# cv-stuttgart/PCFA

Measured on AMD Instinct MI355X. Metric: attack_steps_per_sec, higher is better.
Workload: dtype f32; 1 GPU; RAFT, 1 synthetic 436x1024 pair per GPU (padded 440x1024), disjoint delta, change_of_variables, delta_bound=0.005, zero target, L-BFGS max_iter=10; weights=random:1234, parallelism=pairs sharded 1/GPU, closure_launch=hipGraph replay

## Files before the change

include/pcfa_hip.h:

```cpp
#ifndef PCFA_HIP_H
#define PCFA_HIP_H

#include <stddef.h>
#include <stdint.h>

#ifdef __cplusplus
extern "C" {
#endif

#define PCFA_OK 0
#define PCFA_ERR_INVALID_ARG (-1)
#define PCFA_ERR_UNSUPPORTED (-2)
#define PCFA_ERR_WORKSPACE (-3)

#if defined(__GNUC__)
#define PCFA_API __attribute__((visibility("default")))
#else
#define PCFA_API
#endif

#define PCFA_MAX_LEVELS 8
#define PCFA_ABI_VERSION 3

#define PCFA_LOSS_AEE 0
// ... 224 lines not shown

PCFA_API int pcfa_sepconv5_gru_gates_fwd(const float* h, int C, const float* rest, int Cr, const float* w_packed,
                                const float* add_zr, float* z, float* r, float* rh, int B, int H, int W,
                                int vertical, void* stream);
PCFA_API int pcfa_sepconv5_gru_update_fwd(const float* rh, int C, const float* rest, int Cr, const float* w_packed,
                                 const float* add_q, const float* z, const float* h, float* q, float* hnew, int B,
                                 int H, int W, int vertical, void* stream);
PCFA_API int pcfa_sepconv5_gru_gates_bwd(const float* dqc, int C, int Cr, const float* w_packed_bwd, const float* z,
                                const float* r, const float* h, const float* dz, const float* dh_in, float* dzr,
                                float* dh, float* d_rest, int accumulate_rest, int B, int H, int W, int vertical,
                                void* stream);
PCFA_API int pcfa_sepconv5_gru_update_bwd(const float* dzr, int C, int Cr, const float* w_packed_bwd, const float* dh_acc,
                                 const float* z_prev, const float* q_prev, const float* h_prev, float* dz_prev,
                                 float* dqc_prev, float* dh_prev, float* d_rest, int B, int H, int W, int vertical,
                                 void* stream);

PCFA_API long long pcfa_conv3x3_packed_floats(int K, int N);
PCFA_API int pcfa_conv3x3_pack_weights(const float* w, float* fwd_packed, float* bwd_packed, int Cout, int Cin,
                              void* stream);
PCFA_API int pcfa_conv3x3_fwd(const float* x, const float* packed, const float* bias, float* out, int B, int K, int N,
                     int H, int W, int relu, void* stream);
PCFA_API int pcfa_conv3x3_act_fwd(const float* x, const float* packed, const float* bias, float* out, int B, int K,
                         int N, int H, int W, int act, float slope, void* stream);
PCFA_API int pcfa_leaky_relu_fwd(const float* x, float* y, float slope, long long n, void* stream);
PCFA_API int pcfa_leaky_relu_bwd(const float* out, const float* grad_out, float* grad_x, float slope, long long n,
                        void* stream);
PCFA_API int pcfa_conv3x3_act_fwd_pair(const float* x, const float* packed, const float* bias, float* out, int K, int N,
                              const float* x2, const float* packed2, const float* bias2, float* out2, int K2, int N2,
                              int H, int W, int act, float slope, void* stream);
PCFA_API int pcfa_conv3x3_fused_bwd(const float* g, const float* packed_bwd, const float* mask, const float* addend,
// ... 162 lines not shown
```

pcfa_amd/_hip.py:

```python
import ctypes
import os
from ctypes import c_char_p, c_double, c_float, c_int, c_longlong, c_size_t, c_uint, c_ulonglong, c_void_p, POINTER

ABI_VERSION = 3
LIB_PATH = os.environ.get("PCFA_HIP_LIB") or os.path.join(os.path.dirname(os.path.abspath(__file__)), "lib",
                                                          "libpcfa_hip.so")

PCFA_LOSS = {"aee": 0, "mse": 1, "cosim": 2}


class HipLibraryError(RuntimeError):
    pass


_P = c_void_p
_S4 = POINTER(c_longlong)

SIGNATURES = {
    "pcfa_abi_version": (c_int, []),
    "pcfa_timing_arm": (c_int, [_P, _P, c_int]),
    "pcfa_null_launch": (c_int, [_P]),
    "pcfa_poison_lds": (c_int, [c_uint, _P]),
    "pcfa_peek_lds": (c_int, [_P, c_int, _P]),
    "pcfa_calib_mfma_f32": (c_longlong, [_P, c_int, c_int, _P]),
# ... 79 lines not shown
    "pcfa_sepconv5_algo": (c_int, [c_int]),
    "pcfa_sepconv5_uses_winograd": (c_int, [c_int] * 7),
    "pcfa_sepconv5_pack_weights": (c_int, [_P, _P, _P, c_int, c_int, _P]),
    "pcfa_sepconv5_fwd": (c_int, [_P, c_int, _P, c_int, _P, _P, c_int, c_int, c_int, c_int, c_int, _P]),
    "pcfa_sepconv5_fwd_split": (c_int, [_P, c_int, _P, c_int, _P, _P, c_int, c_int, _P, c_int, c_int, c_int, c_int, c_int,
                                        c_int, _P]),
    "pcfa_gru_gates_bwd_acc": (c_int, [_P, _P, _P, _P, _P, _P, _P, _P, _P, c_longlong, _P]),
    "pcfa_sepconv5_fwd_split_masked": (c_int, [_P, c_int, _P, c_int, _P, _P, c_int, c_int, _P, c_int, _P, c_int, c_int,
                                               c_int, c_int, c_int, c_int, _P]),
    "pcfa_sepconv5_gru_gates_fwd": (c_int, [_P, c_int, _P, c_int, _P, _P, _P, _P, _P, c_int, c_int, c_int, c_int, _P]),
    "pcfa_sepconv5_gru_update_fwd": (c_int, [_P, c_int, _P, c_int, _P, _P, _P, _P, _P, _P, c_int, c_int, c_int, c_int, _P]),
    "pcfa_sepconv5_gru_gates_bwd": (c_int, [_P, c_int, c_int, _P, _P, _P, _P, _P, _P, _P, _P, _P, c_int, c_int, c_int,
                                            c_int, c_int, _P]),
    "pcfa_sepconv5_gru_update_bwd": (c_int, [_P, c_int, c_int, _P, _P, _P, _P, _P, _P, _P, _P, _P, c_int, c_int, c_int,
                                             c_int, _P]),
    "pcfa_convex_upsample_fwd": (c_int, [_P, _P, _P, c_int, c_int, c_int, _P]),
    "pcfa_convex_upsample_workspace_floats": (c_longlong, [c_int, c_int, c_int]),
    "pcfa_convex_upsample_bwd": (c_int, [_P, _P, _P, _P, _P, _P, c_int, c_int, c_int, _P]),
    "pcfa_flow_step": (c_int, [_P, _P, _P, _P, _P, c_longlong, _P]),
    "pcfa_conv3x3_act_fwd_pair": (c_int, [_P, _P, _P, _P, c_int, c_int, _P, _P, _P, _P, c_int, c_int, c_int, c_int, c_int,
                                          c_float, _P]),
    "pcfa_relu_bwd2": (c_int, [_P, _P, _P, _P, _P, c_longlong, _P]),
    "pcfa_conv3x3_fused_bwd": (c_int, [_P, _P, _P, _P, _P, c_int, c_int, c_int, c_int, c_int, _P]),
    "pcfa_conv3x3_masked_fwd": (c_int, [_P, _P, _P, _P, c_int, c_int, c_int, c_int, c_int, _P]),
    "pcfa_conv3x3_algo": (c_int, [c_int] * 5),
    "pcfa_conv3x3_workspace_bytes": (c_size_t, [c_int] * 5),
    "pcfa_conv3x3_run": (c_int, [_P] * 6 + [c_int] * 6 + [c_float, c_int, _P, c_size_t, _P]),
    "pcfa_conv3x3_run_strided": (c_int, [_P, c_longlong, _P, _P, _P, c_longlong, _P, c_longlong, _P, c_longlong]
                                 + [c_int] * 6 + [c_float, c_int, _P, c_size_t, _P]),
    "pcfa_conv3x3_packed_floats": (c_longlong, [c_int, c_int]),
# ... 126 lines not shown
```

pcfa_amd/csrc/gru_math.hip:

```cpp
#include "common.hpp"

namespace {

__device__ __forceinline__ float sigmoidf_(float x) { return 1.0f / (1.0f + expf(-x)); }

template <typename F>
__device__ __forceinline__ void for_each4(long long n, int vec_ok, F f) {
  const long long stride = (long long)gridDim.x * blockDim.x;
  const long long gid = (long long)blockIdx.x * blockDim.x + threadIdx.x;
  if (!vec_ok) {
    for (long long i = gid; i < n; i += stride) f(i, false);
    return;
  }
  const long long n4 = n >> 2;
  for (long long i = gid; i < n4; i += stride) f(i, true);
  if (blockIdx.x == 0 && threadIdx.x < (n & 3)) f((n4 << 2) + threadIdx.x, false);
}

#define LD4(p, i) (*reinterpret_cast<const float4*>((p) + ((i) << 2)))
#define ST4(p, i, v) (*reinterpret_cast<float4*>((p) + ((i) << 2)) = (v))

__device__ __forceinline__ float bias_at(const float* __restrict__ b, long long e, int plane, int C) {
  return b ? b[(e / plane) % C] : 0.f;
}
// ... 80 lines not shown
      o.w = (1.f - zz.w) * hh.w + zz.w * qq.w;
      ST4(q, i, qq); ST4(hnew, i, o);
    } else {
      const float qq = tanhf(qc[i] + (aq ? aq[i] : 0.f) + bias_at(bq, i, plane, C));
      q[i] = qq;
      hnew[i] = (1.f - z[i]) * h[i] + z[i] * qq;
    }
  });
}

__global__ void gru_update_bwd_kernel(const float* __restrict__ z, const float* __restrict__ q,
                                      const float* __restrict__ h, const float* __restrict__ g,
                                      float* __restrict__ dz, float* __restrict__ dqc,
                                      float* __restrict__ dh, long long n, int vec_ok) {
  auto one = [](float z_, float q_, float h_, float g_, float& a, float& b, float& c) {
    a = g_ * q_ - g_ * h_;
    b = (g_ * z_) * (1.f - q_ * q_);
    c = g_ * (1.f - z_);
  };
  for_each4(n, vec_ok, [&](long long i, bool vec) {
    if (vec) {
      const float4 zz = LD4(z, i), qq = LD4(q, i), hh = LD4(h, i), gg = LD4(g, i);
      float4 a, b, c;
      one(zz.x, qq.x, hh.x, gg.x, a.x, b.x, c.x);
      one(zz.y, qq.y, hh.y, gg.y, a.y, b.y, c.y);
      one(zz.z, qq.z, hh.z, gg.z, a.z, b.z, c.z);
      one(zz.w, qq.w, hh.w, gg.w, a.w, b.w, c.w);
      ST4(dz, i, a); ST4(dqc, i, b); ST4(dh, i, c);
    } else {
      one(z[i], q[i], h[i], g[i], dz[i], dqc[i], dh[i]);
    }
  });
}
// ... 199 lines not shown
```

pcfa_amd/csrc/sepconv5.hpp:

```cpp
#pragma once
#include "common.hpp"

namespace pcfa_sc5 {

struct Operand {
  const float* a;
  const float* b;
  int Ca, Cin;
};

struct OutSplit {
  float* a;
  float* b;
  int Ca;
  int acc_a, acc_b;
  const float* mask_b;
  int mask_cb;
};

struct GruEpi {
  int mode, C;
  const float* p0;
  const float* p1;
  const float* p2;
  const float* p3;
  const float* p4;
  float* o0;
  float* o1;
  float* o2;
};

constexpr int PCFA_SC5_NOT_ELIGIBLE = -12345;
int sc5_wino_enabled(int set);
bool sc5_wino_shape_ok(int B, int Cin, int Ca, int Cout, int H, int W, int vertical);
long long sc5_wino_packed_floats(int Cout, int Cin);
int sc5_wino_pack(const float* w, float* packed, int Cout, int Cin, int transpose, hipStream_t stream);
int sc5_wino_launch(const Operand& in, const float* w_wino, const OutSplit& out, int B, int Cout, int H, int W,
                    int vertical, hipStream_t stream, const GruEpi& epi);

}
```

pcfa_amd/csrc/sepconv5_wino.hip:

```cpp
#include <cstdlib>
#include "sepconv5.hpp"

#ifndef PCFA_SC5W_DBG
#define PCFA_SC5W_DBG 0
#endif
#ifndef PCFA_SC5W_WLDS
#define PCFA_SC5W_WLDS 1
#endif
#ifndef PCFA_SC5W_STORE_AT
#define PCFA_SC5W_STORE_AT 1
#endif

namespace {
using namespace pcfa_sc5;

typedef float f32x16 __attribute__((ext_vector_type(16)));
typedef float f32x4 __attribute__((ext_vector_type(4)));
typedef float f32x2 __attribute__((ext_vector_type(2)));

constexpr int CK = 8, STEPS = (CK / 2) * 6;
constexpr int HPX = 128, HRV = HPX / 4 + 2, HCHS = 4 * HRV, HPATCH = CK * HCHS, HNV = CK * HRV;
constexpr int VPX = 64, VCHS = 6 * 64, VPATCH = CK * VCHS, VNV = CK * 6 * 16;

__device__ __attribute__((aligned(16))) float sc5_zero_piece[4] = {0.f, 0.f, 0.f, 0.f};

__device__ __forceinline__ float wino_sigmoid(float x) { return 1.0f / (1.0f + expf(-x)); }

__device__ __forceinline__ const float* wino_plane(const Operand& in, int ci, long long plane) {
  return ci < in.Ca ? in.a + ci * plane : in.b + (ci - in.Ca) * plane;
}

__global__ void sc5_wino_pack_kernel(const float* __restrict__ w, float* __restrict__ P, int N, int C, int transpose,
                                     long long total) {
  const double G[6][5] = {{0.25, 0., 0., 0., 0.},
                          {-1. / 6, -1. / 6, -1. / 6, -1. / 6, -1. / 6},
                          {-1. / 6, 1. / 6, -1. / 6, 1. / 6, -1. / 6},
                          {1. / 24, 2. / 24, 4. / 24, 8. / 24, 16. / 24},
                          {1. / 24, -2. / 24, 4. / 24, -8. / 24, 16. / 24},
                          {0., 0., 0., 0., 1.}};
// ... 5 lines not shown
    const int n = 32 * nb + (lane & 31), c = chunk * CK + 2 * (s / 6) + (lane >> 5), i = s % 6;
    double u = 0.0;
    if (n < N && c < C)
      for (int t = 0; t < 5; ++t)
        u += G[i][t] * (double)(transpose ? w[((long long)c * N + n) * 5 + (4 - t)] : w[((long long)n * C + c) * 5 + t]);
    P[e] = (float)u;
  }
}

template <bool VERT, int WN, int KS, int MODE>
__global__ __launch_bounds__(128 * WN * KS) void sc5_wino_kernel(Operand in, const float* __restrict__ wp, OutSplit out,
                                                                 int Cout, int H, int W, int tiles_x, GruEpi epi) {
  constexpr int GT = 128 * WN, WPG = 2 * WN;
  constexpr int PATCH = VERT ? VPATCH : HPATCH, NV = VERT ? VNV : HNV, NLOAD = (NV + GT - 1) / GT;
  constexpr int RN = 16 / KS;
  constexpr int WBLK = STEPS * 64;
  extern __shared__ __attribute__((aligned(16))) float smem_all[];
  const int grp = __builtin_amdgcn_readfirstlane(threadIdx.x / GT);
  float* smem = smem_all + grp * 2 * PATCH;
  float* wlds = smem_all + KS * 2 * PATCH + grp * 2 * WN * WBLK;
  const int tid = threadIdx.x % GT, lane = tid & 63, l31 = lane & 31, lh = lane >> 5;
  const int wv = __builtin_amdgcn_readfirstlane(tid >> 6);
  const int wn = WN == 2 ? (wv & 1) : 0, wpx = WN == 2 ? (wv >> 1) : wv;
  const int ty = blockIdx.x / tiles_x, x0 = (blockIdx.x - ty * tiles_x) * (VERT ? VPX : HPX);
  const int nb = blockIdx.y * WN + wn;
  const long long plane = (long long)H * W;
  const int nchunk_all = in.Cin / CK, nchunk = nchunk_all / KS;
  in.a += (long long)blockIdx.z * in.Ca * plane;
  if (in.b) in.b += (long long)blockIdx.z * (in.Cin - in.Ca) * plane;
  out.a += (long long)blockIdx.z * out.Ca * plane;
  if (out.b) out.b += (long long)blockIdx.z * (Cout - out.Ca) * plane;
  if (out.mask_b) out.mask_b += (long long)blockIdx.z * (Cout - out.Ca) * plane;

  int poff[NLOAD], pch[NLOAD], plds[NLOAD];
  unsigned okm = 0;
#pragma unroll
  for (int k = 0; k < NLOAD; ++k) {
    const int e = min(tid + GT * k, NV - 1);
    if (VERT) {
      const int c = e / 96, rem = e - c * 96, r = rem >> 4, v = rem & 15;
      const int iy = 2 * ty - 2 + r;
      okm |= (unsigned)((int)(iy >= 0) & (int)(iy < H)) << k;
      poff[k] = min(max(iy, 0), H - 1) * W + x0 + 4 * v;
      pch[k] = c;
      plds[k] = c * VCHS + r * 64 + 4 * v;
    } else {
      const int c = e / HRV, v = e - c * HRV;
// ... 15 lines not shown
      const f32x4 zero = {0.f, 0.f, 0.f, 0.f};
      const f32x4 t = (okm >> k & 1u) ? rr[k] : zero;
      if (tid + GT * k < NV) *reinterpret_cast<f32x4*>(smem + buf * PATCH + plds[k]) = t;
    }
  };
  auto dma_patch = [&](int chunk, int buf) {
#pragma unroll
    for (int k = 0; k < NLOAD; ++k) {
      const float* src = (okm >> k & 1u) ? wino_plane(in, (KS * chunk + grp) * CK + pch[k], plane) + poff[k] : sc5_zero_piece;
      float* dst = smem + buf * PATCH + 4 * (GT * k + 64 * wv);
      if (tid + GT * k < NV)
        __builtin_amdgcn_global_load_lds((const __attribute__((address_space(1))) void*)src,
                                         (__attribute__((address_space(3))) void*)dst, 16, 0, 0);
    }
  };
  const float* pw = wp + ((long long)nb * nchunk_all * STEPS) * 64;

  f32x16 acc[6];
#pragma unroll
  for (int i = 0; i < 6; ++i)
#pragma unroll
    for (int r = 0; r < 16; ++r) acc[i][r] = 0.f;

  f32x4 ra[NLOAD], rb[NLOAD];
  float wa[STEPS], wb[STEPS];
  if (PCFA_SC5W_WLDS) dma_patch(0, 0);
  else load_patch(0, ra);
  auto load_w = [&](int chunk_global, float (&w)[STEPS]) {
    const f32x4* q4 = reinterpret_cast<const f32x4*>(pw + (long long)chunk_global * STEPS * 64);
#pragma unroll
    for (int sq = 0; sq < STEPS / 4; ++sq) {
      const f32x4 t = q4[sq * 64 + lane];
      w[4 * sq] = t.x;
      w[4 * sq + 1] = t.y;
      w[4 * sq + 2] = t.z;
      w[4 * sq + 3] = t.w;
    }
  };
  auto dma_w = [&](int chunk_global, int slot) {
    const float* src = pw + (long long)chunk_global * WBLK + (3 * wpx * 64 + lane) * 4;
    float* dst = wlds + (slot * WN + wn) * WBLK + 3 * wpx * 256;
#pragma unroll
    for (int k = 0; k < 3; ++k)
      __builtin_amdgcn_global_load_lds((const __attribute__((address_space(1))) void*)(src + k * 256),
                                       (__attribute__((address_space(3))) void*)(dst + k * 256), 16, 0, 0);
  };
  auto read_w = [&](int slot, int sq, float (&w)[STEPS]) {
    const f32x4 t = *reinterpret_cast<const f32x4*>(wlds + (slot * WN + wn) * WBLK + (sq * 64 + lane) * 4);
    w[4 * sq] = t.x;
    w[4 * sq + 1] = t.y;
    w[4 * sq + 2] = t.z;
    w[4 * sq + 3] = t.w;
  };
  if (PCFA_SC5W_WLDS) {
    dma_w(grp, 0);
    dma_w(KS * min(1, nchunk - 1) + grp, 1);
  } else {
    load_w(grp, wa);
  }

  const int mw = 32 * nb;
  const bool rowB = !VERT || 2 * ty + 1 < H;
  const long long pix = VERT ? (long long)(2 * ty) * W + x0 + 32 * wpx + l31 : (long long)ty * W + x0 + 64 * wpx + 2 * l31;
  const long long pixB = VERT ? (rowB ? W : 0) : 1;
  const int RB = grp * RN;
  auto ld2 = [&](const float* p, long long idx) -> f32x2 {
    if (!VERT) return *reinterpret_cast<const f32x2*>(p + idx);
    f32x2 v = {p[idx], p[idx + pixB]};
    return v;
  };
  auto st2 = [&](float* p, long long idx, float a, float b) {
    if (!VERT) {
      f32x2 v = {a, b};
      *reinterpret_cast<f32x2*>(p + idx) = v;
    } else {
      p[idx] = a;
      if (rowB) p[idx + W] = b;
    }
  };
  auto ml_of = [&](int rr) { const int r = RB + rr; return (r & 3) + 8 * (r >> 2) + 4 * lh; };

  const bool apart = mw < epi.C;
  f32x2 e0[RN], e1[RN], e2[RN], e3[RN], e4[RN];
#pragma unroll
  for (int rr = 0; rr < RN; ++rr) e0[rr] = e1[rr] = e2[rr] = e3[rr] = e4[rr] = (f32x2){0.f, 0.f};
  if (MODE == 1) {
    const long long ia0 = ((long long)blockIdx.z * 2 * epi.C + mw) * plane + pix;
    const long long ic0 = ((long long)blockIdx.z * epi.C + (apart ? mw : mw - epi.C)) * plane + pix;
#pragma unroll
    for (int rr = 0; rr < RN; ++rr) {
      e0[rr] = ld2(epi.p0, ia0 + ml_of(rr) * plane);
      e1[rr] = ld2(epi.p1, ic0 + ml_of(rr) * plane);
    }
  } else if (MODE == 2) {
    const long long ic0 = ((long long)blockIdx.z * epi.C + mw) * plane + pix;
#pragma unroll
    for (int rr = 0; rr < RN; ++rr) {
      e0[rr] = ld2(epi.p0, ic0 + ml_of(rr) * plane);
      e1[rr] = ld2(epi.p1, ic0 + ml_of(rr) * plane);
      e2[rr] = ld2(epi.p2, ic0 + ml_of(rr) * plane);
    }
  } else if (MODE >= 3) {
    if (apart) {
      const long long ic0 = ((long long)blockIdx.z * epi.C + mw) * plane + pix;
#pragma unroll
      for (int rr = 0; rr < RN; ++rr) {
        e0[rr] = ld2(epi.p0, ic0 + ml_of(rr) * plane);
        e1[rr] = ld2(epi.p1, ic0 + ml_of(rr) * plane);
        e2[rr] = ld2(epi.p2, ic0 + ml_of(rr) * plane);
        e3[rr] = ld2(epi.p3, ic0 + ml_of(rr) * plane);
        if (MODE == 3 && epi.p4 != nullptr) e4[rr] = ld2(epi.p4, ic0 + ml_of(rr) * plane);
      }
    }
  }

  if (PCFA_SC5W_WLDS) asm volatile("s_waitcnt vmcnt(0)" ::: "memory");
  else store_patch(0, ra);
  __syncthreads();
  if (PCFA_SC5W_WLDS) {
#pragma unroll
    for (int sq = 0; sq < STEPS / 4; ++sq) read_w(0, sq, wa);
    __syncthreads();
  } else {
    load_patch(min(1, nchunk - 1), rb);
  }

  const int bl = VERT ? lh * VCHS + 32 * wpx + l31 : lh * HCHS + 2 * (32 * wpx + l31) + 2;
  constexpr int CHS = VERT ? VCHS : HCHS;

// ... 53 lines not shown
          read_w((chunk + 1) & 1, 2 * p + 1, wnext);
        } else {
          read_w((chunk + 1) & 1, p + 2, wnext);
        }
      }
      if (!PCFA_SC5W_WLDS && p == PCFA_SC5W_STORE_AT && !(PCFA_SC5W_DBG & 16)) store_patch((chunk + 1) & 1, rstore);
      __builtin_amdgcn_sched_barrier(0);
    }
    if (!PCFA_SC5W_WLDS && PCFA_SC5W_STORE_AT >= CK / 2 && !(PCFA_SC5W_DBG & 16)) store_patch((chunk + 1) & 1, rstore);
    if (PCFA_SC5W_WLDS) {
      __builtin_amdgcn_sched_barrier(0);
      asm volatile("s_waitcnt vmcnt(0)" ::: "memory");
    }
    if (!(PCFA_SC5W_DBG & 1)) __syncthreads();
  };
  for (int chunk = 0; chunk < nchunk; chunk += 2) {
    item(chunk, wa, wb, ra, rb);
    item(chunk + 1, wb, wa, rb, ra);
  }

  float* sred = smem_all;
#pragma unroll
  for (int r = 0; r < 16; ++r) {
    const float s12 = acc[1][r] + acc[2][r], d12 = acc[1][r] - acc[2][r], s34 = acc[3][r] + acc[4][r],
                d34 = acc[3][r] - acc[4][r];
    sred[((grp * WPG + wv) * 32 + r) * 64 + lane] = acc[0][r] + s12 + s34;
    sred[((grp * WPG + wv) * 32 + 16 + r) * 64 + lane] = fmaf(2.f, d34, d12) + acc[5][r];
  }
  __syncthreads();
  float ya[RN], yb[RN];
#pragma unroll
  for (int rr = 0; rr < RN; ++rr) {
    float sa = 0.f, sb = 0.f;
#pragma unroll
    for (int g = 0; g < KS; ++g) {
      sa += sred[((g * WPG + wv) * 32 + RB + rr) * 64 + lane];
      sb += sred[((g * WPG + wv) * 32 + 16 + RB + rr) * 64 + lane];
    }
    ya[rr] = sa;
    yb[rr] = sb;
  }

  if (MODE == 1) {
    const long long io0 = ((long long)blockIdx.z * epi.C + (apart ? mw : mw - epi.C)) * plane + pix;
#pragma unroll
    for (int rr = 0; rr < RN; ++rr) {
      const long long io = io0 + ml_of(rr) * plane;
      const float sa = wino_sigmoid(ya[rr] + e0[rr].x), sb = wino_sigmoid(yb[rr] + e0[rr].y);
      if (apart) {
        st2(epi.o0, io, sa, sb);
      } else {
        st2(epi.o1, io, sa, sb);
        st2(epi.o2, io, sa * e1[rr].x, sb * e1[rr].y);
      }
    }
  } else if (MODE == 2) {
// ... 20 lines not shown
        const float dr = drh_ * h_;
        ob[q] = dr * (1.f - r_) * r_;
        float c = drh_ * r_;
        if (epi.p4 != nullptr) c += q ? e4[rr].y : e4[rr].x;
        oc[q] = c;
      }
      st2(epi.o0, j0 + ml * plane, oa[0], oa[1]);
      st2(epi.o1, j0 + (long long)(epi.C + ml) * plane, ob[0], ob[1]);
      st2(epi.o2, i0 + ml * plane, oc[0], oc[1]);
    }
  } else if (MODE == 4 && apart) {
    const long long i0 = ((long long)blockIdx.z * epi.C + mw) * plane + pix;
#pragma unroll
    for (int rr = 0; rr < RN; ++rr) {
      const long long i = i0 + ml_of(rr) * plane;
      float oa[2], ob[2], oc[2];
#pragma unroll
      for (int q = 0; q < 2; ++q) {
        const float g_ = (q ? e0[rr].y : e0[rr].x) + (q ? yb[rr] : ya[rr]);
        const float z_ = q ? e1[rr].y : e1[rr].x, q_ = q ? e2[rr].y : e2[rr].x, h_ = q ? e3[rr].y : e3[rr].x;
        oa[q] = g_ * q_ - g_ * h_;
        ob[q] = (g_ * z_) * (1.f - q_ * q_);
        oc[q] = g_ * (1.f - z_);
      }
      st2(epi.o0, i, oa[0], oa[1]);
      st2(epi.o1, i, ob[0], ob[1]);
      st2(epi.o2, i, oc[0], oc[1]);
    }
  } else {
    const bool first = out.b == nullptr || mw < out.Ca;
    float* base = first ? out.a + (long long)mw * plane : out.b + (long long)(mw - out.Ca) * plane;
    const bool accum = first ? out.acc_a != 0 : out.acc_b != 0;
    const bool masked = !first && out.mask_b != nullptr;
    const float* mk = masked ? out.mask_b + (long long)(mw - out.Ca) * plane : base;
#pragma unroll
    for (int rr = 0; rr < RN; ++rr) {
      const int ml = ml_of(rr);
      const long long i = ml * plane + pix;
      float va = ya[rr], vb = yb[rr];
      if (accum) {
        const f32x2 old = ld2(base, i);
        va += old.x;
        vb += old.y;
      }
      if (masked && mw - out.Ca + ml < out.mask_cb) {
        const f32x2 m = ld2(mk, i);
        va = m.x > 0.f ? va : 0.f;
        vb = m.y > 0.f ? vb : 0.f;
      }
      st2(base, i, va, vb);
    }
  }
}

bool wino_aligned16(const void* p) { return (reinterpret_cast<uintptr_t>(p) & 15) == 0; }

template <bool VERT, int WN, int KS, int MODE>
int wino_run(const Operand& in, const float* w, const OutSplit& out, int B, int Cout, int H, int W, hipStream_t s,
             const GruEpi& epi) {
  constexpr int PATCH = VERT ? VPATCH : HPATCH, WPG = 2 * WN;
  constexpr int SRED = KS * WPG * 32 * 64;
  constexpr int STAGE = 2 * KS * PATCH + (PCFA_SC5W_WLDS ? KS * 2 * WN * STEPS * 64 : 0);
  constexpr int LDSF = STAGE > SRED ? STAGE : SRED;
  static bool attr_set = false;
  if (!attr_set) {
    hipError_t e = hipFuncSetAttribute((const void*)sc5_wino_kernel<VERT, WN, KS, MODE>,
                                       hipFuncAttributeMaxDynamicSharedMemorySize, LDSF * (int)sizeof(float));
// ... 71 lines not shown
    }
  } else {
    switch (epi.mode) {
      case 0: PCFA_WINO(false, 0);
      case 1: PCFA_WINO(false, 1);
      case 2: PCFA_WINO(false, 2);
      case 3: PCFA_WINO(false, 3);
      case 4: PCFA_WINO(false, 4);
    }
  }
#undef PCFA_WINO
  return PCFA_SC5_NOT_ELIGIBLE;
}

}
```

pcfa_amd/ops/core.py:

```python
import contextlib
import ctypes
import threading
import weakref

import torch

from .. import _hip

_lane_state = threading.local()
_STREAM_LANE = {}


def current_lane():
    if _STREAM_LANE and torch.cuda.is_available():
        k = _STREAM_LANE.get(torch.cuda.current_stream().cuda_stream)
        if k is not None:
            return k
    return getattr(_lane_state, "k", 0)


@contextlib.contextmanager
def lane(k):
    prev = getattr(_lane_state, "k", 0)
    _lane_state.k = int(k)
# ... 167 lines not shown
    else:
        _note_work("sepconv5_direct", direct, direct)


_WORK_TABLE = {
    "pcfa_conv3x3_run": lambda a: _conv3x3_work(a[6], a[7], a[8], a[9], a[10]),
    "pcfa_conv3x3_act_fwd_pair": lambda a: (_conv3x3_work(1, a[4], a[5], a[12], a[13]),
                                            _conv3x3_work(1, a[10], a[11], a[12], a[13])),
    "pcfa_sepconv5_fwd": lambda a: _sepconv5_work(a[6], a[1], a[3], a[7], a[8], a[9], a[10]),
    "pcfa_sepconv5_fwd_split": lambda a: _sepconv5_work(a[10], a[1], a[3], a[11], a[12], a[13], a[14]),
    "pcfa_sepconv5_fwd_split_masked": lambda a: _sepconv5_work(a[12], a[1], a[3], a[13], a[14], a[15], a[16]),
    "pcfa_sepconv5_gru_gates_fwd": lambda a: _sepconv5_work(a[9], a[1], a[3], 2 * a[1], a[10], a[11], a[12]),
    "pcfa_sepconv5_gru_update_fwd": lambda a: _sepconv5_work(a[10], a[1], a[3], a[1], a[11], a[12], a[13]),
    "pcfa_sepconv5_gru_gates_bwd": lambda a: _sepconv5_work(a[13], a[1], 0, a[1] + a[2], a[14], a[15], a[16]),
    "pcfa_sepconv5_gru_update_bwd": lambda a: _sepconv5_work(a[12], 2 * a[1], 0, a[1] + a[2], a[13], a[14], a[15]),
    "pcfa_instnorm_fwd": lambda a: _note_work("instnorm_fwd", 2.0 * a[4] * a[5] * 4, 0.0),
    "pcfa_instnorm_bwd": lambda a: _note_work("instnorm_bwd", 3.0 * a[5] * a[6] * 4, 0.0),
    "pcfa_conv3x3_fewout_fwd": lambda a: _note_work("conv3x3_fewout_fwd", 4.0 * a[5] * (a[6] + a[7]) * a[8] * a[9], 0.0),
    "pcfa_conv3x3_fewout_bwd": lambda a: _note_work("conv3x3_fewout_bwd", 4.0 * a[4] * (a[5] + a[6]) * a[7] * a[8], 0.0),
    "pcfa_relu_bwd": lambda a: _note_work("relu_bwd", 12.0 * a[3], 0.0),
    "pcfa_relu_bwd2": lambda a: _note_work("relu_bwd2", 20.0 * a[5], 0.0),
    "pcfa_add_relu_fwd": lambda a: _note_work("add_relu_fwd", 12.0 * a[3], 0.0),
    "pcfa_conv_fewin_packed_fwd": lambda a: _note_work("conv_fewin_fwd", *(2 * [2.0 * a[5] * a[9] * a[9] * a[6] * a[4] * a[7] * a[8]])),
}


_spy = None


def set_call_spy(spy):
# ... 53 lines not shown
```

pcfa_amd/ops/gru.py:

```python
import ctypes
import os
import weakref

import torch

from .. import _hip
from . import core
from .core import _call, _dev, _note_work, _pair, _ptr, _ptr_off, _stream
from .conv import _sepconv5_packed, _SepConv5


def _plane_channels(t):
    return t.shape[-2] * t.shape[-1], t.shape[-3]


class _GruGates(torch.autograd.Function):
    @staticmethod
    def forward(ctx, zc, rc, h, bias_z, bias_r, add_z, add_r):
        _dev(zc, rc, h, bias_z, bias_r, add_z, add_r)
        zc, rc, h = zc.contiguous(), rc.contiguous(), h.contiguous()
        az = None if add_z is None else add_z.contiguous()
        ar = None if add_r is None else add_r.contiguous()
        z, r, rh = torch.empty_like(zc), torch.empty_like(zc), torch.empty_like(zc)
        plane, C = _plane_channels(zc)
# ... 84 lines not shown
        plane, C = _plane_channels(x)
        _call("pcfa_bias_relu_fwd", _ptr(x), _ptr(bias), _ptr(out), x.numel(), plane, C)
        ctx.save_for_backward(out)
        return out

    @staticmethod
    def backward(ctx, g):
        (out,) = ctx.saved_tensors
        g = g.contiguous()
        gx = torch.empty_like(out)
        _call("pcfa_relu_bwd", _ptr(out), _ptr(g), _ptr(gx), out.numel())
        return gx, None


_GRU_EPILOGUES = os.environ.get("PCFA_GRU_EPILOGUES", "1") != "0"


class _GruStep(torch.autograd.Function):

    @staticmethod
    def forward(ctx, h, rest, w_zr1, p_zr1, w_q1, p_q1, w_zr2, p_zr2, w_q2, p_q2, rest_relu_channels=0, d_rest_dst=None):
        _dev(h, rest, w_zr1, p_zr1, w_q1, p_q1, w_zr2, p_zr2, w_q2, p_q2)
        h, rest = h.contiguous(), rest.contiguous()
        B, C, H, W = h.shape
        Cr = rest.shape[1]
        n, plane = C * H * W, H * W
        new = lambda c: torch.empty((B, c, H, W), device=h.device, dtype=torch.float32)
        saved, packs = [], []
        for w_zr, p_zr, w_q, p_q in ((w_zr1, p_zr1, w_q1, p_q1), (w_zr2, p_zr2, w_q2, p_q2)):
            if tuple(w_zr.shape[:2]) != (2 * C, C + Cr) or tuple(w_q.shape[:2]) != (C, C + Cr):
                raise ValueError("gru_step: weights %s / %s do not fit h %s, rest %s"
                                 % (tuple(w_zr.shape), tuple(w_q.shape), tuple(h.shape), tuple(rest.shape)))
            vertical = int(w_zr.shape[2] == 5)
            f_zr, b_zr = _sepconv5_packed(w_zr)
            f_q, b_q = _sepconv5_packed(w_q)
            p_zr, p_q = p_zr.contiguous(), p_q.contiguous()
            z, r, rh, q, hnew = new(C), new(C), new(C), new(C), new(C)
# ... 13 lines not shown
                _call("pcfa_sepconv5_fwd", _ptr(rh), C, _ptr(rest), Cr, _ptr(f_q), _ptr(qc), B, C, H, W, vertical)
                _call("pcfa_gru_update_fwd", _ptr(z), _ptr(qc), _ptr(h), None, _ptr(p_q), _ptr(q), _ptr(hnew),
                      z.numel(), plane, C)
            saved += [z, r, q, h]
            packs.append((b_zr, b_q, vertical))
            h = hnew
        ctx.rest_relu = int(rest_relu_channels)
        if not 0 <= ctx.rest_relu <= Cr:
            raise ValueError("gru_step: rest_relu_channels %d outside [0, %d]" % (ctx.rest_relu, Cr))
        ctx.save_for_backward(*saved, *((rest,) if ctx.rest_relu else ()))
        ctx.packs, ctx.dims = packs, (B, C, Cr, H, W)
        if d_rest_dst is not None and (tuple(d_rest_dst.shape) != tuple(rest.shape) or not d_rest_dst.is_contiguous()
                                       or d_rest_dst.dtype != torch.float32 or d_rest_dst.device != rest.device):
            raise ValueError("gru_step: d_rest_dst must be a contiguous float32 tensor of rest's shape %s" % (tuple(rest.shape),))
        ctx.d_rest_dst = d_rest_dst
        return h

    @staticmethod
    def backward(ctx, g):
        if any(ctx.needs_input_grad[i] for i in (2, 4, 6, 8)):
            raise RuntimeError("gru_step is the frozen-weight path: no weight gradient")
        B, C, Cr, H, W = ctx.dims
        n = C * H * W
        new = lambda c: torch.empty((B, c, H, W), device=g.device, dtype=torch.float32)
        g = g.contiguous()
        d_rest = new(Cr) if ctx.d_rest_dst is None else ctx.d_rest_dst
        grads_p = [None, None, None, None]
        if C % 32 == 0 and _GRU_EPILOGUES:
            z1, r1, q1, h1 = ctx.saved_tensors[4:8]
            z0, r0, q0, h0 = ctx.saved_tensors[0:4]
            (b_zr1, b_q1, v1), (b_zr0, b_q0, v0) = ctx.packs[1], ctx.packs[0]
            dz1, dqc1, dh1, dzr1 = new(C), new(C), new(C), new(2 * C)
            _call("pcfa_gru_update_bwd", _ptr(z1), _ptr(q1), _ptr(h1), _ptr(g), _ptr(dz1), _ptr(dqc1), _ptr(dh1), z1.numel())
            _call("pcfa_sepconv5_gru_gates_bwd", _ptr(dqc1), C, Cr, _ptr(b_q1), _ptr(z1), _ptr(r1), _ptr(h1), _ptr(dz1),
                  _ptr(dh1), _ptr(dzr1), _ptr(dh1), _ptr(d_rest), 0, B, H, W, v1)
            dz0, dqc0, dh0, dzr0 = new(C), new(C), new(C), new(2 * C)
            _call("pcfa_sepconv5_gru_update_bwd", _ptr(dzr1), C, Cr, _ptr(b_zr1), _ptr(dh1), _ptr(z0), _ptr(q0), _ptr(h0),
                  _ptr(dz0), _ptr(dqc0), _ptr(dh0), _ptr(d_rest), B, H, W, v1)
            _call("pcfa_sepconv5_gru_gates_bwd", _ptr(dqc0), C, Cr, _ptr(b_q0), _ptr(z0), _ptr(r0), _ptr(h0), _ptr(dz0),
                  _ptr(dh0), _ptr(dzr0), _ptr(dh0), _ptr(d_rest), 1, B, H, W, v0)
            if ctx.rest_relu:
                _call("pcfa_sepconv5_fwd_split_masked", _ptr(dzr0), 2 * C, None, 0, _ptr(b_zr0), _ptr(dh0), C, 1,
                      _ptr(d_rest), 1, _ptr(ctx.saved_tensors[8]), ctx.rest_relu, B, C + Cr, H, W, v0)
            else:
                _call("pcfa_sepconv5_fwd_split", _ptr(dzr0), 2 * C, None, 0, _ptr(b_zr0), _ptr(dh0), C, 1, _ptr(d_rest), 1,
                      B, C + Cr, H, W, v0)
            return dh0, d_rest, None, dzr0, None, dqc0, None, dzr1, None, dqc1, None, None
        rest_started = 0
        for half in (1, 0):
            z, r, q, h = ctx.saved_tensors[4 * half: 4 * half + 4]
            b_zr, b_q, vertical = ctx.packs[half]
            dz, dqc, dh, drh, dzr = new(C), new(C), new(C), new(C), new(2 * C)
            _call("pcfa_gru_update_bwd", _ptr(z), _ptr(q), _ptr(h), _ptr(g), _ptr(dz), _ptr(dqc), _ptr(dh), z.numel())
            _call("pcfa_sepconv5_fwd_split", _ptr(dqc), C, None, 0, _ptr(b_q), _ptr(drh), C, 0, _ptr(d_rest),
                  rest_started, B, C + Cr, H, W, vertical)
            rest_started = 1
# ... 121 lines not shown
```

Measured before the change: 7.908 attack_steps/s.

## Fold next GRU step's update-backward into final sepconv backward epilogue across steps

Adds a new Winograd sepconv5 epilogue mode that, while producing dh for the final conv of one GRU step's backward, also computes the elementwise update-gate backward of the preceding GRU step and stores the accumulated gradient. The preceding step's backward reuses these cached results instead of launching a separate elementwise kernel. This removes one elementwise pass over the hidden-state gradients per GRU iteration. The Winograd kernel is also reworked: weight DMA is issued earlier, epilogue loads are issued after the first chunks, old-value and mask reads are prefetched, and each group reduces its own rows in registers to cut LDS traffic. The cross-step fold depends on autograd producer weakrefs and tensor version checks, which adds fragility.

```diff
diff --git a/include/pcfa_hip.h b/include/pcfa_hip.h
--- a/include/pcfa_hip.h
+++ b/include/pcfa_hip.h
@@ -262,6 +262,10 @@
                                  const float* z_prev, const float* q_prev, const float* h_prev, float* dz_prev,
                                  float* dqc_prev, float* dh_prev, float* d_rest, int B, int H, int W, int vertical,
                                  void* stream);
+PCFA_API int pcfa_sepconv5_gru_update_bwd_next(const float* dzr, int C, int Cr, const float* w_packed_bwd, float* dh,
+                                      const float* z_prev, const float* q_prev, const float* h_prev, float* dz_prev,
+                                      float* dqc_prev, float* dh_prev, float* d_rest, const float* mask_rest,
+                                      int mask_channels, int B, int H, int W, int vertical, void* stream);
 
 PCFA_API long long pcfa_conv3x3_packed_floats(int K, int N);
 PCFA_API int pcfa_conv3x3_pack_weights(const float* w, float* fwd_packed, float* bwd_packed, int Cout, int Cin,
diff --git a/pcfa_amd/_hip.py b/pcfa_amd/_hip.py
--- a/pcfa_amd/_hip.py
+++ b/pcfa_amd/_hip.py
@@ -117,6 +117,8 @@
                                             c_int, c_int, _P]),
     "pcfa_sepconv5_gru_update_bwd": (c_int, [_P, c_int, c_int, _P, _P, _P, _P, _P, _P, _P, _P, _P, c_int, c_int, c_int,
                                              c_int, _P]),
+    "pcfa_sepconv5_gru_update_bwd_next": (c_int, [_P, c_int, c_int, _P, _P, _P, _P, _P, _P, _P, _P, _P, _P, c_int, c_int,
+                                                  c_int, c_int, c_int, _P]),
     "pcfa_convex_upsample_fwd": (c_int, [_P, _P, _P, c_int, c_int, c_int, _P]),
     "pcfa_convex_upsample_workspace_floats": (c_longlong, [c_int, c_int, c_int]),
     "pcfa_convex_upsample_bwd": (c_int, [_P, _P, _P, _P, _P, _P, c_int, c_int, c_int, _P]),
diff --git a/pcfa_amd/csrc/gru_math.hip b/pcfa_amd/csrc/gru_math.hip
--- a/pcfa_amd/csrc/gru_math.hip
+++ b/pcfa_amd/csrc/gru_math.hip
@@ -1,4 +1,5 @@
 #include "common.hpp"
+#include "sepconv5.hpp"
 
 namespace {
 
@@ -118,9 +119,7 @@
                                       float* __restrict__ dz, float* __restrict__ dqc,
                                       float* __restrict__ dh, long long n, int vec_ok) {
   auto one = [](float z_, float q_, float h_, float g_, float& a, float& b, float& c) {
-    a = g_ * q_ - g_ * h_;
-    b = (g_ * z_) * (1.f - q_ * q_);
-    c = g_ * (1.f - z_);
+    pcfa_sc5::gru_update_bwd_math(z_, q_, h_, g_, a, b, c);
   };
   for_each4(n, vec_ok, [&](long long i, bool vec) {
     if (vec) {
diff --git a/pcfa_amd/csrc/sepconv5.hpp b/pcfa_amd/csrc/sepconv5.hpp
--- a/pcfa_amd/csrc/sepconv5.hpp
+++ b/pcfa_amd/csrc/sepconv5.hpp
@@ -28,7 +28,14 @@
   float* o0;
   float* o1;
   float* o2;
+  float* o3;
 };
+
+__device__ __forceinline__ void gru_update_bwd_math(float z, float q, float h, float g, float& dz, float& dqc, float& dh) {
+  dz = g * q - g * h;
+  dqc = (g * z) * (1.f - q * q);
+  dh = g * (1.f - z);
+}
 
 constexpr int PCFA_SC5_NOT_ELIGIBLE = -12345;
 int sc5_wino_enabled(int set);
diff --git a/pcfa_amd/csrc/sepconv5_wino.hip b/pcfa_amd/csrc/sepconv5_wino.hip
--- a/pcfa_amd/csrc/sepconv5_wino.hip
+++ b/pcfa_amd/csrc/sepconv5_wino.hip
@@ -9,6 +9,21 @@
 #endif
 #ifndef PCFA_SC5W_STORE_AT
 #define PCFA_SC5W_STORE_AT 1
+#endif
+#ifndef PCFA_SC5W_EARLY_U
+#define PCFA_SC5W_EARLY_U 1
+#endif
+#ifndef PCFA_SC5W_EARLY_OLD
+#define PCFA_SC5W_EARLY_OLD 1
+#endif
+#ifndef PCFA_SC5W_LATE_EPI
+#define PCFA_SC5W_LATE_EPI 1
+#endif
+#ifndef PCFA_SC5W_OWN_ROWS
+#define PCFA_SC5W_OWN_ROWS 1
+#endif
+#ifndef PCFA_SC5W_STAMPS
+#define PCFA_SC5W_STAMPS 0
 #endif
 
 namespace {
@@ -23,6 +38,20 @@
 constexpr int VPX = 64, VCHS = 6 * 64, VPATCH = CK * VCHS, VNV = CK * 6 * 16;
 
 __device__ __attribute__((aligned(16))) float sc5_zero_piece[4] = {0.f, 0.f, 0.f, 0.f};
+
+#if PCFA_SC5W_STAMPS
+constexpr int SC5W_NSTAMP = 7, SC5W_STAMP_WGS = 1024;
+__device__ unsigned long long sc5w_stamps[SC5W_NSTAMP * SC5W_STAMP_WGS];
+#define SC5W_STAMP(k, drain)                                                              \
+  do {                                                                                    \
+    if (drain) asm volatile("s_waitcnt vmcnt(0) lgkmcnt(0)" ::: "memory");                \
+    __builtin_amdgcn_sched_barrier(0);                                                    \
+    stamp_[k] = __builtin_amdgcn_s_memtime();                                             \
+    __builtin_amdgcn_sched_barrier(0);                                                    \
+  } while (0)
+#else
+#define SC5W_STAMP(k, drain) do { } while (0)
+#endif
 
 __device__ __forceinline__ float wino_sigmoid(float x) { return 1.0f / (1.0f + expf(-x)); }
 
@@ -58,6 +87,7 @@
   constexpr int GT = 128 * WN, WPG = 2 * WN;
   constexpr int PATCH = VERT ? VPATCH : HPATCH, NV = VERT ? VNV : HNV, NLOAD = (NV + GT - 1) / GT;
   constexpr int RN = 16 / KS;
+  constexpr bool EARLY_OLD = PCFA_SC5W_EARLY_OLD && MODE == 0;
   constexpr int WBLK = STEPS * 64;
   extern __shared__ __attribute__((aligned(16))) float smem_all[];
   const int grp = __builtin_amdgcn_readfirstlane(threadIdx.x / GT);
@@ -75,6 +105,25 @@
   out.a += (long long)blockIdx.z * out.Ca * plane;
   if (out.b) out.b += (long long)blockIdx.z * (Cout - out.Ca) * plane;
   if (out.mask_b) out.mask_b += (long long)blockIdx.z * (Cout - out.Ca) * plane;
+#if PCFA_SC5W_STAMPS
+  unsigned long long stamp_[SC5W_NSTAMP];
+  stamp_[5] = __builtin_amdgcn_s_memrealtime();
+#endif
+  SC5W_STAMP(0, false);
+
+  const float* pw = wp + ((long long)nb * nchunk_all * STEPS) * 64;
+  auto dma_w = [&](int chunk_global, int slot) {
+    const float* src = pw + (long long)chunk_global * WBLK + (3 * wpx * 64 + lane) * 4;
+    float* dst = wlds + (slot * WN + wn) * WBLK + 3 * wpx * 256;
+#pragma unroll
+    for (int k = 0; k < 3; ++k)
+      __builtin_amdgcn_global_load_lds((const __attribute__((address_space(1))) void*)(src + k * 256),
+                                       (__attribute__((address_space(3))) void*)(dst + k * 256), 16, 0, 0);
+  };
+  if (PCFA_SC5W_WLDS && PCFA_SC5W_EARLY_U) {
+    dma_w(grp, 0);
+    dma_w(KS * min(1, nchunk - 1) + grp, 1);
+  }
 
   int poff[NLOAD], pch[NLOAD], plds[NLOAD];
   unsigned okm = 0;
@@ -120,7 +169,6 @@
                                          (__attribute__((address_space(3))) void*)dst, 16, 0, 0);
     }
   };
-  const float* pw = wp + ((long long)nb * nchunk_all * STEPS) * 64;
 
   f32x16 acc[6];
 #pragma unroll
@@ -143,14 +191,6 @@
       w[4 * sq + 3] = t.w;
     }
   };
-  auto dma_w = [&](int chunk_global, int slot) {
-    const float* src = pw + (long long)chunk_global * WBLK + (3 * wpx * 64 + lane) * 4;
-    float* dst = wlds + (slot * WN + wn) * WBLK + 3 * wpx * 256;
-#pragma unroll
-    for (int k = 0; k < 3; ++k)
-      __builtin_amdgcn_global_load_lds((const __attribute__((address_space(1))) void*)(src + k * 256),
-                                       (__attribute__((address_space(3))) void*)(dst + k * 256), 16, 0, 0);
-  };
   auto read_w = [&](int slot, int sq, float (&w)[STEPS]) {
     const f32x4 t = *reinterpret_cast<const f32x4*>(wlds + (slot * WN + wn) * WBLK + (sq * 64 + lane) * 4);
     w[4 * sq] = t.x;
@@ -159,8 +199,10 @@
     w[4 * sq + 3] = t.w;
   };
   if (PCFA_SC5W_WLDS) {
-    dma_w(grp, 0);
-    dma_w(KS * min(1, nchunk - 1) + grp, 1);
+    if (!PCFA_SC5W_EARLY_U) {
+      dma_w(grp, 0);
+      dma_w(KS * min(1, nchunk - 1) + grp, 1);
+    }
   } else {
     load_w(grp, wa);
   }
@@ -187,27 +229,32 @@
   auto ml_of = [&](int rr) { const int r = RB + rr; return (r & 3) + 8 * (r >> 2) + 4 * lh; };
 
   const bool apart = mw < epi.C;
+  const bool first = out.b == nullptr || mw < out.Ca;
+  float* base = first ? out.a + (long long)mw * plane : out.b + (long long)(mw - out.Ca) * plane;
+  const bool accum = first ? out.acc_a != 0 : out.acc_b != 0;
+  const bool masked = !first && out.mask_b != nullptr;
+  const float* mk = masked ? out.mask_b + (long long)(mw - out.Ca) * plane : base;
   f32x2 e0[RN], e1[RN], e2[RN], e3[RN], e4[RN];
 #pragma unroll
   for (int rr = 0; rr < RN; ++rr) e0[rr] = e1[rr] = e2[rr] = e3[rr] = e4[rr] = (f32x2){0.f, 0.f};
-  if (MODE == 1) {
-    const long long ia0 = ((long long)blockIdx.z * 2 * epi.C + mw) * plane + pix;
-    const long long ic0 = ((long long)blockIdx.z * epi.C + (apart ? mw : mw - epi.C)) * plane + pix;
-#pragma unroll
-    for (int rr = 0; rr < RN; ++rr) {
-      e0[rr] = ld2(epi.p0, ia0 + ml_of(rr) * plane);
-      e1[rr] = ld2(epi.p1, ic0 + ml_of(rr) * plane);
-    }
-  } else if (MODE == 2) {
-    const long long ic0 = ((long long)blockIdx.z * epi.C + mw) * plane + pix;
-#pragma unroll
-    for (int rr = 0; rr < RN; ++rr) {
-      e0[rr] = ld2(epi.p0, ic0 + ml_of(rr) * plane);
-      e1[rr] = ld2(epi.p1, ic0 + ml_of(rr) * plane);
-      e2[rr] = ld2(epi.p2, ic0 + ml_of(rr) * plane);
-    }
-  } else if (MODE >= 3) {
-    if (apart) {
+  auto request_epi = [&]() {
+    if (MODE == 1) {
+      const long long ia0 = ((long long)blockIdx.z * 2 * epi.C + mw) * plane + pix;
+      const long long ic0 = ((long long)blockIdx.z * epi.C + (apart ? mw : mw - epi.C)) * plane + pix;
+#pragma unroll
+      for (int rr = 0; rr < RN; ++rr) {
+        e0[rr] = ld2(epi.p0, ia0 + ml_of(rr) * plane);
+        e1[rr] = ld2(epi.p1, ic0 + ml_of(rr) * plane);
+      }
+    } else if (MODE == 2) {
+      const long long ic0 = ((long long)blockIdx.z * epi.C + mw) * plane + pix;
+#pragma unroll
+      for (int rr = 0; rr < RN; ++rr) {
+        e0[rr] = ld2(epi.p0, ic0 + ml_of(rr) * plane);
+        e1[rr] = ld2(epi.p1, ic0 + ml_of(rr) * plane);
+        e2[rr] = ld2(epi.p2, ic0 + ml_of(rr) * plane);
+      }
+    } else if (MODE >= 3 && apart) {
       const long long ic0 = ((long long)blockIdx.z * epi.C + mw) * plane + pix;
 #pragma unroll
       for (int rr = 0; rr < RN; ++rr) {
@@ -217,8 +264,16 @@
         e3[rr] = ld2(epi.p3, ic0 + ml_of(rr) * plane);
         if (MODE == 3 && epi.p4 != nullptr) e4[rr] = ld2(epi.p4, ic0 + ml_of(rr) * plane);
       }
-    }
-  }
+    } else if (EARLY_OLD) {
+#pragma unroll
+      for (int rr = 0; rr < RN; ++rr) {
+        const int ml = ml_of(rr);
+        if (accum) e0[rr] = ld2(base, ml * plane + pix);
+        if (masked && mw - out.Ca + ml < out.mask_cb) e1[rr] = ld2(mk, ml * plane + pix);
+      }
+    }
+  };
+  if (!PCFA_SC5W_LATE_EPI) request_epi();
 
   if (PCFA_SC5W_WLDS) asm volatile("s_waitcnt vmcnt(0)" ::: "memory");
   else store_patch(0, ra);
@@ -302,32 +357,77 @@
     }
     if (!(PCFA_SC5W_DBG & 1)) __syncthreads();
   };
-  for (int chunk = 0; chunk < nchunk; chunk += 2) {
+  SC5W_STAMP(1, false);
+  if (PCFA_SC5W_LATE_EPI) {
+    item(0, wa, wb, ra, rb);
+    request_epi();
+    item(1, wb, wa, rb, ra);
+  }
+  for (int chunk = PCFA_SC5W_LATE_EPI ? 2 : 0; chunk < nchunk; chunk += 2) {
     item(chunk, wa, wb, ra, rb);
     item(chunk + 1, wb, wa, rb, ra);
   }
+  SC5W_STAMP(2, false);
 
   float* sred = smem_all;
+  float ta[16], tb[16];
 #pragma unroll
   for (int r = 0; r < 16; ++r) {
     const float s12 = acc[1][r] + acc[2][r], d12 = acc[1][r] - acc[2][r], s34 = acc[3][r] + acc[4][r],
                 d34 = acc[3][r] - acc[4][r];
-    sred[((grp * WPG + wv) * 32 + r) * 64 + lane] = acc[0][r] + s12 + s34;
-    sred[((grp * WPG + wv) * 32 + 16 + r) * 64 + lane] = fmaf(2.f, d34, d12) + acc[5][r];
-  }
-  __syncthreads();
+    ta[r] = acc[0][r] + s12 + s34;
+    tb[r] = fmaf(2.f, d34, d12) + acc[5][r];
+  }
   float ya[RN], yb[RN];
 #pragma unroll
-  for (int rr = 0; rr < RN; ++rr) {
-    float sa = 0.f, sb = 0.f;
-#pragma unroll
-    for (int g = 0; g < KS; ++g) {
-      sa += sred[((g * WPG + wv) * 32 + RB + rr) * 64 + lane];
-      sb += sred[((g * WPG + wv) * 32 + 16 + RB + rr) * 64 + lane];
-    }
-    ya[rr] = sa;
-    yb[rr] = sb;
-  }
+  for (int rr = 0; rr < RN; ++rr) ya[rr] = yb[rr] = 0.f;
+  if (PCFA_SC5W_OWN_ROWS) {
+#pragma unroll
+    for (int G = 0; G < KS; ++G)
+      if (grp == G) {
+#pragma unroll
+        for (int r = 0; r < 16; ++r)
+          if (r < G * RN || r >= (G + 1) * RN) {
+            sred[((G * WPG + wv) * 32 + r) * 64 + lane] = ta[r];
+            sred[((G * WPG + wv) * 32 + 16 + r) * 64 + lane] = tb[r];
+          }
+      }
+    __syncthreads();
+#pragma unroll
+    for (int G = 0; G < KS; ++G)
+      if (grp == G) {
+#pragma unroll
+        for (int rr = 0; rr < RN; ++rr) {
+          float sa = 0.f, sb = 0.f;
+#pragma unroll
+          for (int g = 0; g < KS; ++g) {
+            sa += g == G ? ta[G * RN + rr] : sred[((g * WPG + wv) * 32 + G * RN + rr) * 64 + lane];
+            sb += g == G ? tb[G * RN + rr] : sred[((g * WPG + wv) * 32 + 16 + G * RN + rr) * 64 + lane];
+          }
+          ya[rr] = sa;
+          yb[rr] = sb;
+        }
+      }
+  } else {
+#pragma unroll
+    for (int r = 0; r < 16; ++r) {
+      sred[((grp * WPG + wv) * 32 + r) * 64 + lane] = ta[r];
+      sred[((grp * WPG + wv) * 32 + 16 + r) * 64 + lane] = tb[r];
+    }
+    __syncthreads();
+#pragma unroll
+    for (int rr = 0; rr < RN; ++rr) {
+      float sa = 0.f, sb = 0.f;
+#pragma unroll
+      for (int g = 0; g < KS; ++g) {
+        sa += sred[((g * WPG + wv) * 32 + RB + rr) * 64 + lane];
+        sb += sred[((g * WPG + wv) * 32 + 16 + RB + rr) * 64 + lane];
+      }
+      ya[rr] = sa;
+      yb[rr] = sb;
+    }
+  }
+  SC5W_STAMP(3, true);
 
   if (MODE == 1) {
     const long long io0 = ((long long)blockIdx.z * epi.C + (apart ? mw : mw - epi.C)) * plane + pix;
@@ -378,43 +478,47 @@
 #pragma unroll
     for (int rr = 0; rr < RN; ++rr) {
       const long long i = i0 + ml_of(rr) * plane;
-      float oa[2], ob[2], oc[2];
+      float oa[2], ob[2], oc[2], gg[2];
 #pragma unroll
       for (int q = 0; q < 2; ++q) {
         const float g_ = (q ? e0[rr].y : e0[rr].x) + (q ? yb[rr] : ya[rr]);
         const float z_ = q ? e1[rr].y : e1[rr].x, q_ = q ? e2[rr].y : e2[rr].x, h_ = q ? e3[rr].y : e3[rr].x;
-        oa[q] = g_ * q_ - g_ * h_;
-        ob[q] = (g_ * z_) * (1.f - q_ * q_);
-        oc[q] = g_ * (1.f - z_);
+        gg[q] = g_;
+        gru_update_bwd_math(z_, q_, h_, g_, oa[q], ob[q], oc[q]);
       }
       st2(epi.o0, i, oa[0], oa[1]);
       st2(epi.o1, i, ob[0], ob[1]);
       st2(epi.o2, i, oc[0], oc[1]);
+      if (epi.o3 != nullptr) st2(epi.o3, i, gg[0], gg[1]);
     }
   } else {
-    const bool first = out.b == nullptr || mw < out.Ca;
-    float* base = first ? out.a + (long long)mw * plane : out.b + (long long)(mw - out.Ca) * plane;
-    const bool accum = first ? out.acc_a != 0 : out.acc_b != 0;
-    const bool masked = !first && out.mask_b != nullptr;
-    const float* mk = masked ? out.mask_b + (long long)(mw - out.Ca) * plane : base;
 #pragma unroll
     for (int rr = 0; rr < RN; ++rr) {
       const int ml = ml_of(rr);
       const long long i = ml * plane + pix;
       float va = ya[rr], vb = yb[rr];
       if (accum) {
-        const f32x2 old = ld2(base, i);
+        const f32x2 old = EARLY_OLD ? e0[rr] : ld2(base, i);
         va += old.x;
         vb += old.y;
       }
       if (masked && mw - out.Ca + ml < out.mask_cb) {
-        const f32x2 m = ld2(mk, i);
+        const f32x2 m = EARLY_OLD ? e1[rr] : ld2(mk, i);
         va = m.x > 0.f ? va : 0.f;
         vb = m.y > 0.f ? vb : 0.f;
       }
       st2(base, i, va, vb);
     }
   }
+  SC5W_STAMP(4, true);
+#if PCFA_SC5W_STAMPS
+  stamp_[6] = __builtin_amdgcn_s_memrealtime();
+  const int wg_ = (blockIdx.z * gridDim.y + blockIdx.y) * gridDim.x + blockIdx.x;
+  if (threadIdx.x == 0 && wg_ < SC5W_STAMP_WGS) {
+#pragma unroll
+    for (int k = 0; k < SC5W_NSTAMP; ++k) sc5w_stamps[wg_ * SC5W_NSTAMP + k] = stamp_[k];
+  }
+#endif
 }
 
 bool wino_aligned16(const void* p) { return (reinterpret_cast<uintptr_t>(p) & 15) == 0; }
@@ -516,3 +620,33 @@
 }
 
 }
+
+extern "C" int pcfa_sepconv5_gru_update_bwd_next(const float* dzr, int C, int Cr, const float* w_packed_bwd, float* dh,
+                                                 const float* z_prev, const float* q_prev, const float* h_prev,
+                                                 float* dz_prev, float* dqc_prev, float* dh_prev, float* d_rest,
+                                                 const float* mask_rest, int mask_channels, int B, int H, int W,
+                                                 int vertical, void* stream) {
+  if (!dzr || !w_packed_bwd || !dh || !z_prev || !q_prev || !h_prev || !dz_prev || !dqc_prev || !dh_prev || !d_rest ||
+      C < 32 || C % 32 != 0 || Cr < 1 || B < 1 || H < 1 || W < 1 || mask_channels < 0 || mask_channels > Cr ||
+      (mask_channels > 0 && !mask_rest))
+    return PCFA_ERR_INVALID_ARG;
+  if (dh_prev == dh || dz_prev == dh || dqc_prev == dh) return PCFA_ERR_INVALID_ARG;
+  const int Cin = 2 * C, Cout = C + Cr;
+  if (pcfa_sc5::sc5_wino_packed_floats(Cout, Cin) == 0) return PCFA_ERR_UNSUPPORTED;
+  const pcfa_sc5::Operand in{dzr, nullptr, Cin, Cin};
+  const pcfa_sc5::OutSplit out{dh_prev, d_rest, C, 0, 1, mask_channels > 0 ? mask_rest : nullptr, mask_channels};
+  const pcfa_sc5::GruEpi epi{4, C, dh, z_prev, q_prev, h_prev, nullptr, dz_prev, dqc_prev, dh_prev, dh};
+  const int e = pcfa_sc5::sc5_wino_launch(in, w_packed_bwd + (long long)5 * Cin * Cout, out, B, Cout, H, W, vertical,
+                                          (hipStream_t)stream, epi);
+  return e == pcfa_sc5::PCFA_SC5_NOT_ELIGIBLE ? PCFA_ERR_UNSUPPORTED : e;
+}
+
+#if PCFA_SC5W_STAMPS
+extern "C" __attribute__((visibility("default"))) int pcfa_sc5w_stamps_read(unsigned long long* host, int workgroups) {
+  if (!host || workgroups < 1 || workgroups > SC5W_STAMP_WGS) return PCFA_ERR_INVALID_ARG;
+  hipError_t e = hipDeviceSynchronize();
+  if (e == hipSuccess)
+    e = hipMemcpyFromSymbol(host, HIP_SYMBOL(sc5w_stamps), sizeof(unsigned long long) * SC5W_NSTAMP * workgroups);
+  return (int)e;
+}
+#endif
diff --git a/pcfa_amd/ops/core.py b/pcfa_amd/ops/core.py
--- a/pcfa_amd/ops/core.py
+++ b/pcfa_amd/ops/core.py
@@ -205,6 +205,7 @@
     "pcfa_sepconv5_gru_update_fwd": lambda a: _sepconv5_work(a[10], a[1], a[3], a[1], a[11], a[12], a[13]),
     "pcfa_sepconv5_gru_gates_bwd": lambda a: _sepconv5_work(a[13], a[1], 0, a[1] + a[2], a[14], a[15], a[16]),
     "pcfa_sepconv5_gru_update_bwd": lambda a: _sepconv5_work(a[12], 2 * a[1], 0, a[1] + a[2], a[13], a[14], a[15]),
+    "pcfa_sepconv5_gru_update_bwd_next": lambda a: _sepconv5_work(a[14], 2 * a[1], 0, a[1] + a[2], a[15], a[16], a[17]),
     "pcfa_instnorm_fwd": lambda a: _note_work("instnorm_fwd", 2.0 * a[4] * a[5] * 4, 0.0),
     "pcfa_instnorm_bwd": lambda a: _note_work("instnorm_bwd", 3.0 * a[5] * a[6] * 4, 0.0),
     "pcfa_conv3x3_fewout_fwd": lambda a: _note_work("conv3x3_fewout_fwd", 4.0 * a[5] * (a[6] + a[7]) * a[8] * a[9], 0.0),
diff --git a/pcfa_amd/ops/gru.py b/pcfa_amd/ops/gru.py
--- a/pcfa_amd/ops/gru.py
+++ b/pcfa_amd/ops/gru.py
@@ -122,6 +122,11 @@
 
 
 _GRU_EPILOGUES = os.environ.get("PCFA_GRU_EPILOGUES", "1") != "0"
+_GRU_CHAIN_FOLD = os.environ.get("PCFA_GRU_CHAIN_FOLD", "1") != "0"
+
+
+def _aligned16(*tensors):
+    return all(t.data_ptr() % 16 == 0 for t in tensors)
 
 
 class _GruStep(torch.autograd.Function):
@@ -129,6 +134,7 @@
     @staticmethod
     def forward(ctx, h, rest, w_zr1, p_zr1, w_q1, p_q1, w_zr2, p_zr2, w_q2, p_q2, rest_relu_channels=0, d_rest_dst=None):
         _dev(h, rest, w_zr1, p_zr1, w_q1, p_q1, w_zr2, p_zr2, w_q2, p_q2)
+        producer = h.grad_fn if h.is_contiguous() else None
         h, rest = h.contiguous(), rest.contiguous()
         B, C, H, W = h.shape
         Cr = rest.shape[1]
@@ -172,6 +178,12 @@
                                        or d_rest_dst.dtype != torch.float32 or d_rest_dst.device != rest.device):
             raise ValueError("gru_step: d_rest_dst must be a contiguous float32 tensor of rest's shape %s" % (tuple(rest.shape),))
         ctx.d_rest_dst = d_rest_dst
+        ctx.fold_ok = C % 32 == 0 and _GRU_EPILOGUES and _GRU_CHAIN_FOLD
+        ctx.folded = None
+        ctx.producer = None
+        if (ctx.fold_ok and isinstance(producer, _GruStep._backward_cls) and getattr(producer, "fold_ok", False)
+                and (producer.dims[0], producer.dims[1]) + producer.dims[3:] == (B, C, H, W)):
+            ctx.producer = weakref.ref(producer)
         return h
 
     @staticmethod
@@ -188,8 +200,16 @@
             z1, r1, q1, h1 = ctx.saved_tensors[4:8]
             z0, r0, q0, h0 = ctx.saved_tensors[0:4]
             (b_zr1, b_q1, v1), (b_zr0, b_q0, v0) = ctx.packs[1], ctx.packs[0]
-            dz1, dqc1, dh1, dzr1 = new(C), new(C), new(C), new(2 * C)
-            _call("pcfa_gru_update_bwd", _ptr(z1), _ptr(q1), _ptr(h1), _ptr(g), _ptr(dz1), _ptr(dqc1), _ptr(dh1), z1.numel())
+            dzr1 = new(2 * C)
+            folded, ctx.folded = ctx.folded, None
+            if (folded is not None and g.data_ptr() == folded[0].data_ptr() and g.shape == folded[0].shape
+                    and g._version == folded[1]):
+                dz1, dqc1, dh1 = folded[2:]
+            else:
+                dz1, dqc1, dh1 = new(C), new(C), new(C)
+                _call("pcfa_gru_update_bwd", _ptr(z1), _ptr(q1), _ptr(h1), _ptr(g), _ptr(dz1), _ptr(dqc1), _ptr(dh1),
+                      z1.numel())
+            folded = None
             _call("pcfa_sepconv5_gru_gates_bwd", _ptr(dqc1), C, Cr, _ptr(b_q1), _ptr(z1), _ptr(r1), _ptr(h1), _ptr(dz1),
                   _ptr(dh1), _ptr(dzr1), _ptr(dh1), _ptr(d_rest), 0, B, H, W, v1)
             dz0, dqc0, dh0, dzr0 = new(C), new(C), new(C), new(2 * C)
@@ -197,7 +217,16 @@
                   _ptr(dz0), _ptr(dqc0), _ptr(dh0), _ptr(d_rest), B, H, W, v1)
             _call("pcfa_sepconv5_gru_gates_bwd", _ptr(dqc0), C, Cr, _ptr(b_q0), _ptr(z0), _ptr(r0), _ptr(h0), _ptr(dz0),
                   _ptr(dh0), _ptr(dzr0), _ptr(dh0), _ptr(d_rest), 1, B, H, W, v0)
-            if ctx.rest_relu:
+            prod = ctx.producer() if ctx.producer is not None else None
+            if (prod is not None and _aligned16(dzr0, dh0, d_rest)
+                    and _hip.load().pcfa_sepconv5_uses_winograd(B, 2 * C, 0, C + Cr, H, W, v0)):
+                zp, _, qp, hp = prod.saved_tensors[4:8]
+                dzp, dqcp, dhp = new(C), new(C), new(C)
+                _call("pcfa_sepconv5_gru_update_bwd_next", _ptr(dzr0), C, Cr, _ptr(b_zr0), _ptr(dh0), _ptr(zp), _ptr(qp),
+                      _ptr(hp), _ptr(dzp), _ptr(dqcp), _ptr(dhp), _ptr(d_rest),
+                      _ptr(ctx.saved_tensors[8]) if ctx.rest_relu else None, ctx.rest_relu, B, H, W, v0)
+                prod.folded = (dh0, dh0._version, dzp, dqcp, dhp)
+            elif ctx.rest_relu:
                 _call("pcfa_sepconv5_fwd_split_masked", _ptr(dzr0), 2 * C, None, 0, _ptr(b_zr0), _ptr(dh0), C, 1,
                       _ptr(d_rest), 1, _ptr(ctx.saved_tensors[8]), ctx.rest_relu, B, C + Cr, H, W, v0)
             else:
```

After: 7.894 attack_steps/s. No clear change (-0.2%).
